# treangenlab/Seqwin

Hardware: AMD Instinct MI355X
Metric: Gbp/s minimizer-indexed (higher is better)
Workload: dtype u64

## Files before the change

### seqwin_amd/csrc/radix.hip

```cpp
#include <algorithm>
#include <cstdlib>
#include <cstring>
#include <vector>
#include <map>
#include <mutex>

#include "device.hpp"

namespace sw {
namespace {

constexpr int RS_ITEMS = 16;
#ifdef SW_RS_STAMPS
__device__ unsigned long long *g_rs_stamps = nullptr;
#define RS_STAMP(i)                                                                                        \
    do {                                                                                                   \
        if (g_rs_stamps && (tile & 63u) == 0 && threadIdx.x == 0) g_rs_stamps[(size_t)(tile >> 6) * 16 + (i)] = clock64(); \
    } while (0)
#else
#define RS_STAMP(i) do { } while (0)
#endif
#ifndef RS_LOOK
#define RS_LOOK 4
#endif
// ... 1098 lines not shown

bool radix_unsort_perm(uint64_t *&keys, uint64_t *&alt, uint64_t n, unsigned low_bits, unsigned nbit, hipStream_t stream, uint32_t *d_fail)
{
    constexpr int THREADS = 512, BITS = 8;
    constexpr uint32_t RADIX = 1u << BITS, TILE = THREADS * RS_ITEMS;
    if (n == 0 || nbit <= low_bits + 8 || nbit > low_bits + 16 || SW_AB_GETENV("SEQWIN_AMD_RADIX_STABLE_UNSORT")) return false;
    if ((1ull << (low_bits + 8)) % TILE) return false;
    const char *kind = SW_AB_GETENV("SEQWIN_AMD_RADIX_KERNEL");
    if (kind && !strcmp(kind, "classic")) return false;
    const unsigned hi_bits = nbit - low_bits - 8;
    const uint32_t n_groups = (uint32_t)((n + (1ull << (low_bits + 8)) - 1) >> (low_bits + 8));
    const uint64_t n_tiles = (n + TILE - 1) / TILE;
    int dev = 0, per_cu = 0;
    SW_HIP(hipGetDevice(&dev));
    hipDeviceProp_t prop;
    SW_HIP(hipGetDeviceProperties(&prop, dev));
    SW_HIP(hipOccupancyMaxActiveBlocksPerMultiprocessor(&per_cu, k_rs_pass_p<THREADS, BITS, 0>, THREADS, 0));
    const unsigned grid = (unsigned)std::min<uint64_t>(n_tiles, (uint64_t)std::max(1, per_cu) * std::max(1, prop.multiProcessorCount));
    DevArray<unsigned long long> cur_a((size_t)RADIX * RS_CURSOR_STRIDE), cur_b((size_t)n_groups * RADIX);
    DevArray<uint32_t> tickets(2);
    SW_HIP(hipMemsetAsync(tickets.p, 0, 8, stream));
    hipLaunchKernelGGL(k_rs_perm_cursors, dim3(1), dim3(RADIX), 0, stream, cur_a.p, 1u, RADIX, RS_CURSOR_STRIDE, 64u, low_bits + 8);
    hipLaunchKernelGGL(k_rs_perm_cursors, dim3((n_groups * RADIX + 255) / 256), dim3(256), 0, stream, cur_b.p, n_groups, RADIX, 1u,
                       low_bits + 8, low_bits);
    auto pass = ballot_forced() ? k_rs_pass_p<THREADS, BITS, 0> : k_rs_pass_p<THREADS, BITS, 1>;
    hipLaunchKernelGGL(pass, dim3(grid), dim3(THREADS), 0, stream, (const uint64_t *)keys, alt, n, (uint32_t)n_tiles,
                       32u + low_bits + 8, hi_bits, (const unsigned long long *)nullptr, (unsigned long long *)nullptr, tickets.p, d_fail,
                       0u, cur_a.p, RS_CURSOR_STRIDE, 64u, 0u);
    std::swap(keys, alt);
    hipLaunchKernelGGL(pass, dim3(grid), dim3(THREADS), 0, stream, (const uint64_t *)keys, alt, n, (uint32_t)n_tiles, 32u + low_bits,
                       8u, (const unsigned long long *)nullptr, (unsigned long long *)nullptr, tickets.p + 1, d_fail, 0u, cur_b.p, 1u,
                       low_bits + 8, 0u);
    std::swap(keys, alt);
    SW_HIP(hipGetLastError());
    return true;
}

bool radix_pairs_available() { return rank_mode() == 1; }
int radix_rank_mode() { return rank_mode(); }

uint64_t radix_trim_state()
{
    uint64_t freed = 0;
    if (g_state_uses) return 0;
    std::lock_guard<std::mutex> lock(state_registry_mu());
    for (auto &kv : state_registry()) {
        StateBuf &b = *kv.second;
        std::unique_lock<std::mutex> use(b.mu, std::try_to_lock);
        if (!use.owns_lock() || !b.p) continue;
        int cur = -1;
        (void)hipGetDevice(&cur);
        if (cur != kv.first.first) (void)hipSetDevice(kv.first.first);
        (void)hipFree(b.p);
        if (cur != kv.first.first && cur >= 0) (void)hipSetDevice(cur);
        freed += b.words * 8;
        b.p = nullptr;
        b.words = 0;
        b.epoch = 0;
    }
    return freed;
}

void radix_demote_rank()
{
    int dev = 0;
    SW_HIP(hipGetDevice(&dev));
    std::lock_guard<std::mutex> lock(rank_mu());
    rank_modes()[dev] = 0;
}

void radix_sort_pairs32(uint32_t *&keys, uint32_t *&keys_alt, OccPay *&vals, OccPay *&vals_alt, uint64_t n, unsigned end_bit,
                        hipStream_t stream, uint32_t *d_fail, const StageSource *src, const std::function<void()> &after_first,
                        uint32_t *low_out)
{
    constexpr uint32_t RADIX = 1u << RP_BITS, TILE = RP_THREADS * RP_ITEMS;
    if (n == 0 || end_bit == 0) return;
    if (end_bit > 32 || end_bit % RP_BITS) raise(SW_ERR_RUNTIME, "radix_sort_pairs32: key bits must be a multiple of 8 up to 32");
    if (n >= 0xFFFFFFFFull) raise(SW_ERR_RUNTIME, "radix_sort_pairs32: more than 2^32-2 elements");
    const unsigned n_passes = end_bit / RP_BITS;
    const uint64_t n_tiles = (n + TILE - 1) / TILE;
    int grid_p = 0;
    {
        static std::mutex &mu = *new std::mutex;
        static std::map<int, int> &grids = *new std::map<int, int>;
        int dev = 0;
        SW_HIP(hipGetDevice(&dev));
        std::lock_guard<std::mutex> lock(mu);
        int &g = grids[dev];
        if (!g) {
            int per_cu = 0;
            hipDeviceProp_t prop;
            SW_HIP(hipGetDeviceProperties(&prop, dev));
            SW_HIP(hipOccupancyMaxActiveBlocksPerMultiprocessor(&per_cu, k_rs_pair_pass<0>, RP_THREADS, 0));
            g = std::max(1, per_cu) * std::max(1, prop.multiProcessorCount);
        }
        grid_p = g;
    }
    DevArray<unsigned long long> hist((size_t)n_passes * RADIX);
    DevArray<uint32_t> tickets(n_passes);
    SW_HIP(hipMemsetAsync(tickets.p, 0, tickets.bytes(), stream));
    SW_HIP(hipMemsetAsync(hist.p, 0, hist.bytes(), stream));
    StageSource stage{};
    DevArray<uint32_t> chunk_tile;
    DevArray<unsigned long long> chunk_dir;
    if (src && src->rows) {
        stage = *src;
        hipLaunchKernelGGL(k_rs_hist32_rows, dim3((unsigned)((n + 16383) / 16384)), dim3(256), 0, stream,
                           reinterpret_cast<const uint4 *>(src->rows), n, n_passes, hist.p);
    } else if (src) {
        constexpr uint64_t CHUNK = 64 * RP_ITEMS;
        static_assert(TILE == (RP_THREADS / 64) * CHUNK, "a tile is one chunk per wave");
        const uint64_t n_chunks = (n + CHUNK - 1) / CHUNK;
        stage = *src;
        chunk_tile.alloc(n_chunks);
        chunk_dir.alloc(n_chunks * STAGE_ROW);
        stage.chunk_dir = chunk_dir.p;
        hipLaunchKernelGGL(k_rs_chunk_tiles, dim3((stage.n_tiles + 255u) / 256u), dim3(256), 0, stream, stage.tile_count, stage.dst_off,
                           stage.n_tiles, chunk_tile.p);
        hipLaunchKernelGGL(k_rs_stage_prepare, dim3((unsigned)std::min<uint64_t>(2048, (n_chunks + 3) / 4)), dim3(256), 0, stream, stage,
                           (const uint32_t *)chunk_tile.p, n, n_passes, chunk_dir.p, hist.p);
    } else {
        hipLaunchKernelGGL(k_rs_hist32, dim3((unsigned)((n + 65535) / 65536)), dim3(256), 0, stream, keys, n, n_passes, hist.p);
    }
    SW_HIP(hipGetLastError());
    StateUse su = state_buf(stream, (size_t)n_tiles * RADIX);
    StateBuf &sb = su.b;
    const StageSource none{};
    const uint32_t fault = fault_rank();
    for (unsigned p = 0; p < n_passes; ++p) {
        hipLaunchKernelGGL(k_rs_scan<RP_BITS>, dim3(1), dim3(RADIX), 0, stream, hist.p + (size_t)p * RADIX, (unsigned long long *)nullptr);
        const uint32_t epoch = next_epoch(sb, stream);
        const dim3 grid((unsigned)std::min<uint64_t>(n_tiles, (uint64_t)grid_p));
        if (p == 0 && src) {
            auto first = src->rows ? k_rs_pair_pass<2> : k_rs_pair_pass<1>;
            hipLaunchKernelGGL(first, grid, dim3(RP_THREADS), 0, stream, (const uint32_t *)nullptr, (const uint4 *)nullptr,
                               keys_alt, reinterpret_cast<uint4 *>(vals_alt), n, (uint32_t)n_tiles, 0u,
                               (const unsigned long long *)hist.p, sb.p, epoch, tickets.p, d_fail, stage,
                               n_passes == 1 ? low_out : (uint32_t *)nullptr, fault);
            SW_HIP(hipGetLastError());
            if (after_first) after_first();
        } else {
            hipLaunchKernelGGL(k_rs_pair_pass<0>, grid, dim3(RP_THREADS), 0, stream, (const uint32_t *)keys,
                               reinterpret_cast<const uint4 *>(vals), keys_alt, reinterpret_cast<uint4 *>(vals_alt), n, (uint32_t)n_tiles,
                               RP_BITS * p, (const unsigned long long *)(hist.p + (size_t)p * RADIX), sb.p, epoch, tickets.p + p, d_fail,
                               none, p + 1 == n_passes ? low_out : (uint32_t *)nullptr, fault);
            SW_HIP(hipGetLastError());
        }
        std::swap(keys, keys_alt);
        std::swap(vals, vals_alt);
    }
}

namespace {
constexpr uint32_t EB_RADIX = 512, EB_TABLE = EB_RADIX * EB_RADIX, EB_THREADS = 512;
constexpr uint64_t EB_EMPTY = ~0ull;
static_assert(EB_THREADS == EB_RADIX, "k_eb_finish: one bin per thread");
enum : uint32_t { EB_F_OVERFLOW = 1u, EB_F_RANGE = 2u, EB_F_ORDER = 4u };
struct EbInfo {
    unsigned long long n_sentinels;
    uint32_t n_tiles2, max_bucket, flags, n_runs;
};

__global__ __launch_bounds__(EB_RADIX) void k_eb_level1(const unsigned long long *__restrict__ h1, uint32_t tile_keys,
                                                        unsigned long long *__restrict__ cursor, unsigned long long *__restrict__ segtab,
                                                        EbInfo *__restrict__ info)
{
    __shared__ unsigned long long s[EB_RADIX];
    __shared__ uint32_t st[EB_RADIX];
    const uint32_t d = threadIdx.x;
    const unsigned long long c = h1[d];
    const uint32_t tiles = (uint32_t)((c + tile_keys - 1) / tile_keys);
    s[d] = c;
    st[d] = tiles;
    __syncthreads();
    for (uint32_t o = 1; o < EB_RADIX; o <<= 1) {
        const unsigned long long a = d >= o ? s[d - o] : 0;
        const uint32_t b = d >= o ? st[d - o] : 0;
        __syncthreads();
        s[d] += a;
        st[d] += b;
        __syncthreads();
    }
    const unsigned long long first = s[d] - c;
    cursor[(size_t)d * RS_CURSOR_STRIDE] = first;
    uint32_t w = st[d] - tiles;
    for (uint32_t t = 0; t < tiles; ++t)
        segtab[w + t] = seg_pack(first + (uint64_t)t * tile_keys, d, (uint32_t)min((unsigned long long)tile_keys, c - (uint64_t)t * tile_keys));
    if (d == EB_RADIX - 1) info->n_tiles2 = st[d];
}

__global__ __launch_bounds__(1024) void k_eb_count(const uint64_t *__restrict__ in, const unsigned long long *__restrict__ segtab,
                                                   const EbInfo *__restrict__ info, unsigned shift, uint32_t dmask, uint64_t sentinel,
                                                   uint32_t *__restrict__ table, EbInfo *__restrict__ out)
{
    __shared__ uint32_t hist[EB_RADIX];
    __shared__ uint32_t s_sent;
    const uint32_t n_tiles = info->n_tiles2;
    for (uint32_t w = blockIdx.x; w < n_tiles; w += gridDim.x) {
        const unsigned long long seg = segtab[w];
        const uint64_t first = seg_first(seg);
        const uint32_t cnt = seg_count(seg);
        if (threadIdx.x < EB_RADIX) hist[threadIdx.x] = 0;
        if (threadIdx.x == 0) s_sent = 0;
        __syncthreads();
        uint64_t key[RS_ITEMS];
#pragma unroll
        for (int i = 0; i < RS_ITEMS; ++i) {
            const uint32_t li = i * 1024 + threadIdx.x;
            key[i] = li < cnt ? in[first + li] : EB_EMPTY;
        }
        uint32_t sent = 0;
#pragma unroll
        for (int i = 0; i < RS_ITEMS; ++i) {
            if (key[i] == EB_EMPTY) continue;
            if (key[i] == sentinel) ++sent;
            atomicAdd(&hist[(uint32_t)(key[i] >> shift) & dmask], 1u);
        }
        if (sent) atomicAdd(&s_sent, sent);
        __syncthreads();
        if (threadIdx.x < EB_RADIX && hist[threadIdx.x]) atomicAdd(&table[seg_bucket(seg) * EB_RADIX + threadIdx.x], hist[threadIdx.x]);
        if (threadIdx.x == 0 && s_sent) atomicAdd(&out->n_sentinels, (unsigned long long)s_sent);
        __syncthreads();
    }
}

__global__ __launch_bounds__(1024) void k_eb_scan(const uint32_t *__restrict__ cnt, const unsigned long long *__restrict__ n_sent,
                                                  uint32_t sent_at, uint32_t *__restrict__ start, unsigned long long *__restrict__ cursor,
                                                  uint32_t *__restrict__ max_out, uint32_t *__restrict__ total_out)
{
    constexpr uint32_t PER4 = EB_TABLE / 1024 / 4;
    __shared__ uint32_t ws[16], wm[16];
    const uint32_t tid = threadIdx.x, lane = tid & 63u, wave = tid >> 6;
    const uint32_t sent = n_sent ? (uint32_t)*n_sent : 0u;
    const uint4 *cnt4 = reinterpret_cast<const uint4 *>(cnt) + (size_t)tid * PER4;
    uint32_t sum = 0, mx = 0;
#pragma unroll 16
    for (uint32_t j = 0; j < PER4; ++j) {
        const uint4 c = cnt4[j];
        mx = max(max(max(mx, c.x), max(c.y, c.z)), c.w);
        sum += c.x + c.y + c.z + c.w;
    }
    if (n_sent && sent_at / (4 * PER4) == tid) {
        mx = 0;
        for (uint32_t j = 0; j < 4 * PER4; ++j) {
            const uint32_t i = tid * 4 * PER4 + j, c = cnt[i];
            mx = max(mx, c - (i == sent_at ? min(c, sent) : 0u));
        }
    }
    uint32_t incl = sum;
    for (uint32_t o = 1; o < 64; o <<= 1) {
        const uint32_t up = __shfl_up(incl, o, 64);
        if (lane >= o) incl += up;
        mx = max(mx, __shfl_xor(mx, o, 64));
    }
    if (lane == 63) ws[wave] = incl;
    if (lane == 0) wm[wave] = mx;
    __syncthreads();
    uint32_t run = incl - sum;
    for (uint32_t w = 0; w < wave; ++w) run += ws[w];
    uint4 *start4 = reinterpret_cast<uint4 *>(start) + (size_t)tid * PER4;
    ulonglong2 *cur2 = reinterpret_cast<ulonglong2 *>(cursor) + (size_t)tid * PER4 * 2;
#pragma unroll 16
    for (uint32_t j = 0; j < PER4; ++j) {
        const uint4 c = cnt4[j];
        const uint4 st = make_uint4(run, run + c.x, run + c.x + c.y, run + c.x + c.y + c.z);
        start4[j] = st;
        if (cursor) {
            cur2[2 * j] = make_ulonglong2(st.x, st.y);
            cur2[2 * j + 1] = make_ulonglong2(st.z, st.w);
        }
        run = st.w + c.w;
    }
    if (tid == 1023) {
        start[EB_TABLE] = run;
        if (total_out) *total_out = run;
        uint32_t m = 0;
        for (uint32_t w = 0; w < 16; ++w) m = max(m, wm[w]);
        if (max_out) *max_out = m;
    }
}

__global__ __launch_bounds__(EB_THREADS) void k_eb_finish(const uint64_t *__restrict__ in, const uint32_t *__restrict__ start, uint32_t slots,
                                                          unsigned shift1, unsigned shift2, uint32_t mask2, unsigned bin_shift,
                                                          uint32_t bin_mask, uint64_t sentinel,
                                                          uint64_t *__restrict__ tk, uint32_t *__restrict__ tc,
                                                          uint32_t *__restrict__ n_distinct, uint32_t *__restrict__ flags)
{
    extern __shared__ __align__(16) unsigned char eb_lds[];
    unsigned long long *hk = reinterpret_cast<unsigned long long *>(eb_lds);
    uint32_t *hc = reinterpret_cast<uint32_t *>(hk + slots);
    uint16_t *idx = reinterpret_cast<uint16_t *>(hc + slots);
    __shared__ uint32_t bd[EB_RADIX + 1], bk[EB_RADIX], bcur[EB_RADIX], wsd[EB_THREADS / 64], wsk[EB_THREADS / 64];
    __shared__ uint32_t s_over;
    const uint32_t b = EB_TABLE - 1u - blockIdx.x, tid = threadIdx.x, lane = tid & 63u, wave = tid >> 6;
    const uint32_t first = start[b], cnt = start[b + 1] - first;
    if (cnt == 0) return;
    const uint32_t mask = slots - 1u;
    for (uint32_t s = tid; s < slots; s += EB_THREADS) {
        hk[s] = EB_EMPTY;
        hc[s] = 0;
    }
    bd[tid] = 0;
    bk[tid] = 0;
    if (tid == 0) s_over = 0;
    __syncthreads();
    uint32_t bad = 0;
    for (uint32_t j0 = 0; j0 < cnt; j0 += 4 * EB_THREADS) {
        if (*(volatile uint32_t *)&s_over) break;
        uint64_t key[4];
#pragma unroll
        for (int i = 0; i < 4; ++i) {
            const uint32_t j = j0 + i * EB_THREADS + tid;
            key[i] = j < cnt ? in[(uint64_t)first + j] : sentinel;
        }
#pragma unroll
        for (int i = 0; i < 4; ++i) {
            uint64_t k = key[i];
            bool live = k != sentinel;
            if (live && ((uint32_t)(k >> shift1) * EB_RADIX + ((uint32_t)(k >> shift2) & mask2)) != b) {
                bad = 1;
                live = false;
            }
            uint32_t copies = 1;
            const uint64_t any = __ballot(live);
            if (any) {
                const int src = __ffsll((long long)any) - 1;
                const uint64_t k0 = (uint64_t)__shfl((unsigned long long)k, src, 64);
                const uint64_t same = __ballot(live && k == k0);
                if (live && k == k0) {
                    copies = (uint32_t)__popcll(same);
                    live = (int)lane == src;
                }
            }
            if (!live) continue;
            uint32_t h = (uint32_t)((k * 0x9E3779B97F4A7C15ull) >> 40) & mask, probes = 0;
            for (; probes < slots; ++probes) {
                const unsigned long long old = atomicCAS(&hk[h], EB_EMPTY, (unsigned long long)k);
                if (old == EB_EMPTY || old == k) {
                    atomicAdd(&hc[h], copies);
                    break;
                }
                h = (h + 1u) & mask;
            }
            if (probes == slots) s_over = 1;
        }
    }
    if (bad) atomicOr(flags, EB_F_RANGE);
    __syncthreads();
    if (s_over) {
        if (tid == 0) atomicOr(flags, EB_F_OVERFLOW);
        return;
    }
    for (uint32_t s = tid; s < slots; s += EB_THREADS) {
        const uint64_t k = hk[s];
        if (k == EB_EMPTY) continue;
        const uint32_t bin = (uint32_t)(k >> bin_shift) & bin_mask;
        atomicAdd(&bd[bin], 1u);
        atomicAdd(&bk[bin], hc[s]);
    }
    __syncthreads();
    {
        const uint32_t d = bd[tid], c = bk[tid];
        uint32_t id = d, ic = c;
        for (uint32_t o = 1; o < 64; o <<= 1) {
            const uint32_t ud = __shfl_up(id, o, 64), uc = __shfl_up(ic, o, 64);
            if (lane >= o) {
                id += ud;
                ic += uc;
            }
        }
        if (lane == 63) {
            wsd[wave] = id;
            wsk[wave] = ic;
        }
        __syncthreads();
        uint32_t pd = id - d, pc = ic - c;
        for (uint32_t w = 0; w < wave; ++w) {
            pd += wsd[w];
            pc += wsk[w];
        }
        bd[tid] = pd;
        bcur[tid] = pd;
        bk[tid] = pc;
        if (tid == EB_THREADS - 1) bd[EB_RADIX] = pd + d;
    }
    __syncthreads();
    for (uint32_t s = tid; s < slots; s += EB_THREADS) {
        const uint64_t k = hk[s];
        if (k == EB_EMPTY) continue;
        idx[atomicAdd(&bcur[(uint32_t)(k >> bin_shift) & bin_mask], 1u)] = (uint16_t)s;
    }
    __syncthreads();
    const uint32_t n_dist = bd[EB_RADIX];
    if (tid == 0) n_distinct[b] = n_dist;
    for (uint32_t j = tid; j < n_dist; j += EB_THREADS) {
        const uint32_t s = idx[j];
        const uint64_t k = hk[s];
        const uint32_t bin = (uint32_t)(k >> bin_shift) & bin_mask, lo = bd[bin], hi = bd[bin + 1];
        uint32_t less = 0, copies_less = 0;
        for (uint32_t i = lo; i < hi; ++i) {
            const uint32_t s2 = idx[i];
            if (hk[s2] < k) {
                ++less;
                copies_less += hc[s2];
            }
        }
        tk[(uint64_t)first + lo + less] = k;
        tc[(uint64_t)first + lo + less] = first + bk[bin] + copies_less;
    }
}

__global__ __launch_bounds__(256) void k_eb_compact(const uint64_t *__restrict__ tk, const uint32_t *__restrict__ tc,
                                                    const uint32_t *__restrict__ start, const uint32_t *__restrict__ dstart,
                                                    const unsigned long long *__restrict__ n_sentinels, uint64_t *__restrict__ ukeys,
                                                    uint32_t *__restrict__ ucnt, uint32_t *__restrict__ flags)
{
    const uint32_t b = blockIdx.x, d0 = dstart[b], n = dstart[b + 1] - d0;
    if (b == EB_TABLE - 1u && threadIdx.x == 0) ucnt[dstart[EB_TABLE]] = start[EB_TABLE] - (uint32_t)*n_sentinels;
    if (n == 0) return;
    const uint64_t first = start[b];
    uint32_t bad = 0;
    for (uint32_t j = threadIdx.x; j < n; j += 256) {
        const uint64_t k = tk[first + j];
        const uint32_t c = tc[first + j];
        if (j + 1 < n && (tk[first + j + 1] <= k || tc[first + j + 1] <= c)) bad = 1;
        if (c < first || c >= start[b + 1]) bad = 1;
        ukeys[d0 + j] = k;
        ucnt[d0 + j] = c;
    }
    if (bad) atomicOr(flags, EB_F_ORDER);
}
}

int radix_edge_buckets(uint64_t *&keys, uint64_t *&alt, uint64_t m, unsigned key_bits, uint64_t sentinel,
                       const unsigned long long *d_hist_top, uint32_t cap, uint32_t slots, uint64_t *ukeys, uint32_t *ucnt,
                       uint32_t *n_runs, hipStream_t stream, uint32_t *d_fail, bool debug)
{
    constexpr int THREADS = 1024, BITS = 9;
    constexpr uint32_t TILE = THREADS * RS_ITEMS;
    unsigned digit_bits = 0, n_passes = 0;
    radix_layout(key_bits, &digit_bits, &n_passes);
    if (n_passes < 2 || m >= (1ull << 32) - 1 || slots < 64 || slots > 8192 || (slots & (slots - 1))) return 1;
    const unsigned shift1 = (n_passes - 1) * digit_bits, bits1 = key_bits - shift1;
    const unsigned bits2 = std::min<unsigned>(BITS, shift1), shift2 = shift1 - bits2;
    const unsigned bin_bits = std::min<unsigned>(BITS, shift2), bin_shift = shift2 - bin_bits;
    const uint64_t n_tiles = (m + TILE - 1) / TILE, max_tiles2 = n_tiles + EB_RADIX;
    int dev = 0, per_cu = 0;
    SW_HIP(hipGetDevice(&dev));
    hipDeviceProp_t prop;
    SW_HIP(hipGetDeviceProperties(&prop, dev));
    SW_HIP(hipOccupancyMaxActiveBlocksPerMultiprocessor(&per_cu, k_rs_pass_p<THREADS, BITS, 0>, THREADS, 0));
    const unsigned cus = (unsigned)std::max(1, prop.multiProcessorCount);
    const unsigned grid = (unsigned)std::min<uint64_t>(n_tiles, (uint64_t)std::max(1, per_cu) * cus);

    DevArray<unsigned long long> h1(EB_RADIX), cur1((size_t)EB_RADIX * RS_CURSOR_STRIDE), cur2(EB_TABLE), segtab(max_tiles2);
    DevArray<uint32_t> table(EB_TABLE), start(EB_TABLE + 1), tickets(2), flags(1);
    DevArray<EbInfo> info(1);
    SW_HIP(hipMemsetAsync(h1.p, 0, h1.bytes(), stream));
    SW_HIP(hipMemsetAsync(table.p, 0, table.bytes(), stream));
    SW_HIP(hipMemsetAsync(tickets.p, 0, 8, stream));
    SW_HIP(hipMemsetAsync(flags.p, 0, 4, stream));
    SW_HIP(hipMemsetAsync(info.p, 0, sizeof(EbInfo), stream));
    if (d_hist_top)
        SW_HIP(hipMemcpyAsync(h1.p, d_hist_top, (size_t)8 << digit_bits, hipMemcpyDeviceToDevice, stream));
    else
        hipLaunchKernelGGL(k_rs_hist<BITS>, dim3((unsigned)((m + 32767) / 32768)), dim3(256), 0, stream, (const uint64_t *)keys, m, shift1,
                           key_bits, 1u, h1.p);
    hipLaunchKernelGGL(k_eb_level1, dim3(1), dim3(EB_RADIX), 0, stream, (const unsigned long long *)h1.p, TILE, cur1.p, segtab.p, info.p);
    auto pass1 = ballot_forced() ? k_rs_pass_p<THREADS, BITS, 0> : k_rs_pass_p<THREADS, BITS, 1>;
    hipLaunchKernelGGL(pass1, dim3(grid), dim3(THREADS), 0, stream, (const uint64_t *)keys, alt, m, (uint32_t)n_tiles, shift1, bits1,
                       (const unsigned long long *)nullptr, (unsigned long long *)nullptr, tickets.p, d_fail, 0u, cur1.p, RS_CURSOR_STRIDE,
                       64u, 0u);
    std::swap(keys, alt);
    hipLaunchKernelGGL(k_eb_count, dim3((unsigned)std::min<uint64_t>(max_tiles2, (uint64_t)8 * cus)), dim3(1024), 0, stream,
                       (const uint64_t *)keys, (const unsigned long long *)segtab.p, (const EbInfo *)info.p, shift2, (1u << bits2) - 1u,
                       sentinel, table.p, info.p);
    const uint32_t sent_at = (uint32_t)(sentinel >> shift1) * EB_RADIX + ((uint32_t)(sentinel >> shift2) & ((1u << bits2) - 1u));
    hipLaunchKernelGGL(k_eb_scan, dim3(1), dim3(1024), 0, stream, (const uint32_t *)table.p, (const unsigned long long *)&info.p->n_sentinels,
                       sent_at, start.p, cur2.p, &info.p->max_bucket, (uint32_t *)nullptr);
    SW_HIP(hipGetLastError());
    EbInfo hi;
    SW_HIP(hipMemcpyAsync(&hi, info.p, sizeof hi, hipMemcpyDeviceToHost, stream));
    SW_HIP(hipStreamSynchronize(stream));
    if (debug)
        fprintf(stderr, "[edge buckets] %llu keys, %llu sentinels, digits %u+%u+%u of %u bits, largest sub-bucket %u (capacity %u, %u slots)%s\n",
                (unsigned long long)m, hi.n_sentinels, bits1, bits2, bin_bits, key_bits, hi.max_bucket, cap, slots,
                hi.max_bucket > cap ? ": radix passes instead" : "");
    if (hi.max_bucket > cap) return 1;
    auto pass2 = ballot_forced() ? k_rs_pass_p<THREADS, BITS, 0, true> : k_rs_pass_p<THREADS, BITS, 1, true>;
    hipLaunchKernelGGL(pass2, dim3(std::max(1u, std::min(hi.n_tiles2, (uint32_t)(std::max(1, per_cu) * cus)))), dim3(THREADS), 0, stream,
                       (const uint64_t *)keys, alt, m, hi.n_tiles2, shift2, bits2, (const unsigned long long *)segtab.p,
                       (unsigned long long *)nullptr, tickets.p + 1, d_fail, 0u, cur2.p, 1u, 64u, 0u);
    std::swap(keys, alt);
    DevArray<uint32_t> tc(m), n_distinct(EB_TABLE), dstart(EB_TABLE + 1);
    SW_HIP(hipMemsetAsync(n_distinct.p, 0, n_distinct.bytes(), stream));
    uint64_t *tk = alt;
    const size_t lds = (size_t)slots * 14;
    static std::mutex &mu = *new std::mutex;
    {
        std::lock_guard<std::mutex> lock(mu);
        SW_HIP(hipFuncSetAttribute(reinterpret_cast<const void *>(k_eb_finish), hipFuncAttributeMaxDynamicSharedMemorySize, (int)lds));
    }
    hipLaunchKernelGGL(k_eb_finish, dim3(EB_TABLE), dim3(EB_THREADS), lds, stream, (const uint64_t *)keys, (const uint32_t *)start.p, slots,
                       shift1, shift2, (1u << bits2) - 1u, bin_shift, (1u << bin_bits) - 1u, sentinel, tk, tc.p, n_distinct.p, flags.p);
    hipLaunchKernelGGL(k_eb_scan, dim3(1), dim3(1024), 0, stream, (const uint32_t *)n_distinct.p, (const unsigned long long *)nullptr, 0u,
                       dstart.p, (unsigned long long *)nullptr, (uint32_t *)nullptr, &info.p->n_runs);
    hipLaunchKernelGGL(k_eb_compact, dim3(EB_TABLE), dim3(256), 0, stream, (const uint64_t *)tk, (const uint32_t *)tc.p,
                       (const uint32_t *)start.p, (const uint32_t *)dstart.p, (const unsigned long long *)&info.p->n_sentinels, ukeys, ucnt,
                       flags.p);
    SW_HIP(hipGetLastError());
    uint32_t hf = 0;
    SW_HIP(hipMemcpyAsync(&hi, info.p, sizeof hi, hipMemcpyDeviceToHost, stream));
    SW_HIP(hipMemcpyAsync(&hf, flags.p, 4, hipMemcpyDeviceToHost, stream));
    SW_HIP(hipStreamSynchronize(stream));
    if (hf & (EB_F_RANGE | EB_F_ORDER))
        raise(SW_ERR_RUNTIME, "internal error: the edge buckets are out of order (%s)", hf & EB_F_RANGE ? "a key outside its bucket" : "run starts descend");
    if (hf & EB_F_OVERFLOW) {
        if (debug) fprintf(stderr, "[edge buckets] a sub-bucket holds more than %u distinct keys: radix passes instead\n", slots);
        return 1;
    }
    *n_runs = hi.n_runs;
    return 0;
}

static int pick_shape(unsigned bits)
{
    const char *e = SW_TEST_GETENV("SEQWIN_AMD_RADIX_BITS");
    const bool nine = e ? atoi(e) == 9 : (bits + 8) / 9 < (bits + 7) / 8;
    const char *shape = SW_AB_GETENV("SEQWIN_AMD_RADIX_SHAPE");
    if (shape && !strcmp(shape, "1024x8")) return 2;
    if (shape && !strcmp(shape, "512x9")) return 3;
    if (shape && !strcmp(shape, "256x8")) return 4;
    return nine ? 1 : 0;
}

void radix_layout(unsigned bits, unsigned *digit_bits, unsigned *n_passes)
{
    const int sh = pick_shape(bits);
    *digit_bits = (sh == 1 || sh == 3) ? 9u : 8u;
    *n_passes = (bits + *digit_bits - 1) / *digit_bits;
}

void radix_sort_keys64(uint64_t *&keys, uint64_t *&alt, uint64_t n, unsigned begin_bit, unsigned end_bit, hipStream_t stream,
                       uint32_t *d_fail, bool perm_hi32, unsigned long long *d_hist_given, unsigned layout_bits)
{
    if (n == 0 || end_bit <= begin_bit) return;
    if (end_bit - begin_bit > 64) raise(SW_ERR_RUNTIME, "radix_sort_keys64: more than 64 key bits");
    switch (pick_shape(layout_bits ? layout_bits : end_bit - begin_bit)) {
#ifdef SW_AB
    case 2: sort_passes<1024, 8>(keys, alt, n, begin_bit, end_bit, stream, d_fail, perm_hi32, d_hist_given); break;
    case 3: sort_passes<512, 9>(keys, alt, n, begin_bit, end_bit, stream, d_fail, perm_hi32, d_hist_given); break;
    case 4: sort_passes<256, 8>(keys, alt, n, begin_bit, end_bit, stream, d_fail, perm_hi32, d_hist_given); break;
#endif
    case 1: sort_passes<1024, 9>(keys, alt, n, begin_bit, end_bit, stream, d_fail, perm_hi32, d_hist_given); break;
    default: sort_passes<512, 8>(keys, alt, n, begin_bit, end_bit, stream, d_fail, perm_hi32, d_hist_given); break;
    }
}

}
```

Baseline: 474.5.

## Size edge-bucket finish hash tables by bucket class with persistent ticketed workgroups

```diff
diff --git a/seqwin_amd/csrc/radix.hip b/seqwin_amd/csrc/radix.hip
--- a/seqwin_amd/csrc/radix.hip
+++ b/seqwin_amd/csrc/radix.hip
@@ -1274,14 +1274,18 @@
 }
 
 namespace {
-constexpr uint32_t EB_RADIX = 512, EB_TABLE = EB_RADIX * EB_RADIX, EB_THREADS = 512;
+constexpr uint32_t EB_RADIX = 512, EB_TABLE = EB_RADIX * EB_RADIX;
 constexpr uint64_t EB_EMPTY = ~0ull;
-static_assert(EB_THREADS == EB_RADIX, "k_eb_finish: one bin per thread");
 enum : uint32_t { EB_F_OVERFLOW = 1u, EB_F_RANGE = 2u, EB_F_ORDER = 4u };
 struct EbInfo {
     unsigned long long n_sentinels;
     uint32_t n_tiles2, max_bucket, flags, n_runs;
 };
+constexpr uint32_t EB_MAX_CLASSES = 3;
+struct EbClasses {
+    uint32_t n, slots[EB_MAX_CLASSES], bound[EB_MAX_CLASSES], max_keys[EB_MAX_CLASSES];
+};
+enum : uint32_t { EB_CTL_COUNT = 0, EB_CTL_TICKET = 4, EB_CTL_PROMOTED = 8, EB_CTL_WORDS = 12 };
 
 __global__ __launch_bounds__(EB_RADIX) void k_eb_level1(const unsigned long long *__restrict__ h1, uint32_t tile_keys,
                                                         unsigned long long *__restrict__ cursor, unsigned long long *__restrict__ segtab,
@@ -1402,133 +1406,255 @@
     }
 }
 
-__global__ __launch_bounds__(EB_THREADS) void k_eb_finish(const uint64_t *__restrict__ in, const uint32_t *__restrict__ start, uint32_t slots,
-                                                          unsigned shift1, unsigned shift2, uint32_t mask2, unsigned bin_shift,
-                                                          uint32_t bin_mask, uint64_t sentinel,
-                                                          uint64_t *__restrict__ tk, uint32_t *__restrict__ tc,
-                                                          uint32_t *__restrict__ n_distinct, uint32_t *__restrict__ flags)
-{
+#ifdef SW_EB_STAMPS
+constexpr uint32_t EB_STAMP_N = 4096, EB_STAMP_W = 12;
+__device__ unsigned long long g_eb_stamps[EB_MAX_CLASSES][EB_STAMP_N][EB_STAMP_W];
+#define EB_STAMP_SET(t) const uint32_t stamp_at = ((t) & 15u) == 0 && ((t) >> 4) < EB_STAMP_N && threadIdx.x == 0 ? ((t) >> 4) : ~0u
+#define EB_STAMP(i) do { if (stamp_at != ~0u) g_eb_stamps[cls][stamp_at][i] = clock64(); } while (0)
+#define EB_STAMP_END(cnt, nd) do { if (stamp_at != ~0u) { g_eb_stamps[cls][stamp_at][9] = clock64(); g_eb_stamps[cls][stamp_at][10] = (cnt); g_eb_stamps[cls][stamp_at][11] = (nd); } } while (0)
+#else
+#define EB_STAMP_SET(t) do { } while (0)
+#define EB_STAMP(i) do { } while (0)
+#define EB_STAMP_END(cnt, nd) do { } while (0)
+#endif
+__global__ __launch_bounds__(1024) void k_eb_classify(const uint32_t *__restrict__ start, EbClasses cl, uint32_t force,
+                                                      uint4 *__restrict__ lists, uint32_t *__restrict__ ctl)
+{
+    const uint32_t b = (blockIdx.x ? blockIdx.x - 1u : gridDim.x - 1u) * 1024u + threadIdx.x, lane = threadIdx.x & 63u;
+    const uint32_t first = start[b], cnt = start[b + 1] - first;
+    uint32_t mine = EB_MAX_CLASSES;
+    if (cnt) {
+        mine = 0;
+        while (mine + 1 < cl.n && cnt > cl.max_keys[mine]) ++mine;
+        if (force < cl.n) mine = force;
+    }
+    for (uint32_t c = 0; c < cl.n; ++c) {
+        const uint64_t in = __ballot(mine == c);
+        if (!in) continue;
+        const int leader = __ffsll((long long)in) - 1;
+        uint32_t base = 0;
+        if ((int)lane == leader) base = atomicAdd(&ctl[EB_CTL_COUNT + c], (uint32_t)__popcll(in));
+        base = __shfl(base, leader, 64);
+        if (mine == c) lists[(size_t)c * EB_TABLE + base + (uint32_t)__popcll(in & ((1ull << lane) - 1ull))] = make_uint4(first, cnt, b, 0u);
+    }
+}
+
+template <int THREADS, bool ONE>
+__global__ __launch_bounds__(THREADS) void k_eb_finish(const uint64_t *__restrict__ in, uint4 *lists, uint32_t *__restrict__ ctl,
+                                                       uint32_t cls, EbClasses cl, unsigned shift1, unsigned shift2, uint32_t mask2,
+                                                       unsigned bin_shift, uint32_t bin_mask, unsigned cbits, uint64_t sentinel,
+                                                       uint64_t *__restrict__ tk, uint32_t *__restrict__ tc,
+                                                       uint32_t *__restrict__ n_distinct, uint32_t *__restrict__ flags)
+{
+    constexpr uint32_t BPT = EB_RADIX / THREADS, TILE = 4 * THREADS;
+    static_assert(BPT * THREADS == EB_RADIX, "k_eb_finish: whole bins per thread");
     extern __shared__ __align__(16) unsigned char eb_lds[];
+    const uint32_t slots = cl.slots[cls], bound = cl.bound[cls], mask = slots - 1u;
     unsigned long long *hk = reinterpret_cast<unsigned long long *>(eb_lds);
     uint32_t *hc = reinterpret_cast<uint32_t *>(hk + slots);
-    uint16_t *idx = reinterpret_cast<uint16_t *>(hc + slots);
-    __shared__ uint32_t bd[EB_RADIX + 1], bk[EB_RADIX], bcur[EB_RADIX], wsd[EB_THREADS / 64], wsk[EB_THREADS / 64];
-    __shared__ uint32_t s_over;
-    const uint32_t b = EB_TABLE - 1u - blockIdx.x, tid = threadIdx.x, lane = tid & 63u, wave = tid >> 6;
-    const uint32_t first = start[b], cnt = start[b + 1] - first;
-    if (cnt == 0) return;
-    const uint32_t mask = slots - 1u;
-    for (uint32_t s = tid; s < slots; s += EB_THREADS) {
-        hk[s] = EB_EMPTY;
-        hc[s] = 0;
-    }
-    bd[tid] = 0;
-    bk[tid] = 0;
-    if (tid == 0) s_over = 0;
-    __syncthreads();
-    uint32_t bad = 0;
-    for (uint32_t j0 = 0; j0 < cnt; j0 += 4 * EB_THREADS) {
-        if (*(volatile uint32_t *)&s_over) break;
-        uint64_t key[4];
+    uint16_t *idx = ONE ? reinterpret_cast<uint16_t *>(hk + slots) : reinterpret_cast<uint16_t *>(hc + slots);
+    __shared__ uint32_t bd[EB_RADIX + 1], bk[EB_RADIX], bcur[EB_RADIX], wsd[THREADS / 64], wsk[THREADS / 64];
+    __shared__ uint32_t s_over, s_ticket;
+    const uint32_t tid = threadIdx.x, lane = tid & 63u, wave = tid >> 6;
+    const uint64_t cmask = (1ull << cbits) - 1ull, low = (1ull << shift2) - 1ull;
+    auto slot_key = [&](uint32_t s) -> uint64_t { return ONE ? hk[s] >> cbits : hk[s]; };
+    auto slot_copies = [&](uint32_t s) -> uint32_t { return ONE ? (uint32_t)(hk[s] & cmask) : hc[s]; };
+    const uint4 *list = lists + (size_t)cls * EB_TABLE;
+    const uint32_t n_list = ctl[EB_CTL_COUNT + cls];
+    if (tid == 0) s_ticket = atomicAdd(&ctl[EB_CTL_TICKET + cls], 1u);
+    __syncthreads();
+    uint32_t t = s_ticket;
+    uint4 work = make_uint4(0u, 0u, 0u, 0u);
+    uint64_t key[4] = {sentinel, sentinel, sentinel, sentinel};
+    if (t < n_list) {
+        work = list[t];
 #pragma unroll
         for (int i = 0; i < 4; ++i) {
-            const uint32_t j = j0 + i * EB_THREADS + tid;
-            key[i] = j < cnt ? in[(uint64_t)first + j] : sentinel;
-        }
-#pragma unroll
-        for (int i = 0; i < 4; ++i) {
-            uint64_t k = key[i];
-            bool live = k != sentinel;
-            if (live && ((uint32_t)(k >> shift1) * EB_RADIX + ((uint32_t)(k >> shift2) & mask2)) != b) {
-                bad = 1;
-                live = false;
-            }
-            uint32_t copies = 1;
-            const uint64_t any = __ballot(live);
-            if (any) {
-                const int src = __ffsll((long long)any) - 1;
-                const uint64_t k0 = (uint64_t)__shfl((unsigned long long)k, src, 64);
-                const uint64_t same = __ballot(live && k == k0);
-                if (live && k == k0) {
-                    copies = (uint32_t)__popcll(same);
-                    live = (int)lane == src;
+            const uint32_t j = i * THREADS + tid;
+            key[i] = j < work.y ? in[(uint64_t)work.x + j] : sentinel;
+        }
+    }
+    __syncthreads();
+    while (t < n_list) {
+        const uint32_t first = work.x, cnt = work.y, b = work.z;
+        EB_STAMP_SET(t);
+        EB_STAMP(0);
+        const uint64_t high = ((uint64_t)(b / EB_RADIX) << shift1) | ((uint64_t)(b % EB_RADIX) << shift2);
+        for (uint32_t s = tid; s < slots; s += THREADS) {
+            hk[s] = EB_EMPTY;
+            if (!ONE) hc[s] = 0;
+        }
+#pragma unroll
+        for (uint32_t i = 0; i < BPT; ++i) {
+            bd[i * THREADS + tid] = 0;
+            bk[i * THREADS + tid] = 0;
+        }
+        if (tid == 0) {
+            s_over = 0;
+            s_ticket = atomicAdd(&ctl[EB_CTL_TICKET + cls], 1u);
+        }
+        __syncthreads();
+        EB_STAMP(1);
+        uint32_t bad = 0;
+        for (uint32_t j0 = 0;;) {
+#pragma unroll
+            for (int i = 0; i < 4; ++i) {
+                uint64_t k = key[i];
+                bool live = k != sentinel;
+                if (live && ((uint32_t)(k >> shift1) * EB_RADIX + ((uint32_t)(k >> shift2) & mask2)) != b) {
+                    bad = 1;
+                    live = false;
                 }
-            }
-            if (!live) continue;
-            uint32_t h = (uint32_t)((k * 0x9E3779B97F4A7C15ull) >> 40) & mask, probes = 0;
-            for (; probes < slots; ++probes) {
-                const unsigned long long old = atomicCAS(&hk[h], EB_EMPTY, (unsigned long long)k);
-                if (old == EB_EMPTY || old == k) {
-                    atomicAdd(&hc[h], copies);
-                    break;
+                uint32_t copies = 1;
+                const uint64_t any = __ballot(live);
+                if (any) {
+                    const int src = __ffsll((long long)any) - 1;
+                    const uint64_t k0 = (uint64_t)__shfl((unsigned long long)k, src, 64);
+                    const uint64_t same = __ballot(live && k == k0);
+                    if (live && k == k0) {
+                        copies = (uint32_t)__popcll(same);
+                        live = (int)lane == src;
+                    }
                 }
-                h = (h + 1u) & mask;
-            }
-            if (probes == slots) s_over = 1;
-        }
-    }
-    if (bad) atomicOr(flags, EB_F_RANGE);
-    __syncthreads();
-    if (s_over) {
-        if (tid == 0) atomicOr(flags, EB_F_OVERFLOW);
-        return;
-    }
-    for (uint32_t s = tid; s < slots; s += EB_THREADS) {
-        const uint64_t k = hk[s];
-        if (k == EB_EMPTY) continue;
-        const uint32_t bin = (uint32_t)(k >> bin_shift) & bin_mask;
-        atomicAdd(&bd[bin], 1u);
-        atomicAdd(&bk[bin], hc[s]);
-    }
-    __syncthreads();
-    {
-        const uint32_t d = bd[tid], c = bk[tid];
-        uint32_t id = d, ic = c;
-        for (uint32_t o = 1; o < 64; o <<= 1) {
-            const uint32_t ud = __shfl_up(id, o, 64), uc = __shfl_up(ic, o, 64);
-            if (lane >= o) {
-                id += ud;
-                ic += uc;
-            }
-        }
-        if (lane == 63) {
-            wsd[wave] = id;
-            wsk[wave] = ic;
-        }
+                if (!live) continue;
+                uint32_t h = (uint32_t)((k * 0x9E3779B97F4A7C15ull) >> 40) & mask, probes = 0;
+                if (ONE) {
+                    const uint64_t rem = k & low;
+                    const unsigned long long fresh = (unsigned long long)((rem << cbits) | copies);
+                    for (; probes < slots; ++probes) {
+                        const unsigned long long old = atomicCAS(&hk[h], EB_EMPTY, fresh);
+                        if (old == EB_EMPTY) break;
+                        if ((old >> cbits) == rem) {
+                            atomicAdd(&hk[h], (unsigned long long)copies);
+                            break;
+                        }
+                        h = (h + 1u) & mask;
+                    }
+                } else {
+                    for (; probes < slots; ++probes) {
+                        const unsigned long long old = atomicCAS(&hk[h], EB_EMPTY, (unsigned long long)k);
+                        if (old == EB_EMPTY || old == k) {
+                            atomicAdd(&hc[h], copies);
+                            break;
+                        }
+                        h = (h + 1u) & mask;
+                    }
+                }
+                if (probes == slots) s_over = 1;
+            }
+            j0 += TILE;
+            if (j0 >= cnt || *(volatile uint32_t *)&s_over) break;
+#pragma unroll
+            for (int i = 0; i < 4; ++i) {
+                const uint32_t j = j0 + i * THREADS + tid;
+                key[i] = j < cnt ? in[(uint64_t)first + j] : sentinel;
+            }
+        }
+        if (bad) atomicOr(flags, EB_F_RANGE);
+        EB_STAMP(2);
         __syncthreads();
-        uint32_t pd = id - d, pc = ic - c;
-        for (uint32_t w = 0; w < wave; ++w) {
-            pd += wsd[w];
-            pc += wsk[w];
-        }
-        bd[tid] = pd;
-        bcur[tid] = pd;
-        bk[tid] = pc;
-        if (tid == EB_THREADS - 1) bd[EB_RADIX] = pd + d;
-    }
-    __syncthreads();
-    for (uint32_t s = tid; s < slots; s += EB_THREADS) {
-        const uint64_t k = hk[s];
-        if (k == EB_EMPTY) continue;
-        idx[atomicAdd(&bcur[(uint32_t)(k >> bin_shift) & bin_mask], 1u)] = (uint16_t)s;
-    }
-    __syncthreads();
-    const uint32_t n_dist = bd[EB_RADIX];
-    if (tid == 0) n_distinct[b] = n_dist;
-    for (uint32_t j = tid; j < n_dist; j += EB_THREADS) {
-        const uint32_t s = idx[j];
-        const uint64_t k = hk[s];
-        const uint32_t bin = (uint32_t)(k >> bin_shift) & bin_mask, lo = bd[bin], hi = bd[bin + 1];
-        uint32_t less = 0, copies_less = 0;
-        for (uint32_t i = lo; i < hi; ++i) {
-            const uint32_t s2 = idx[i];
-            if (hk[s2] < k) {
-                ++less;
-                copies_less += hc[s2];
-            }
-        }
-        tk[(uint64_t)first + lo + less] = k;
-        tc[(uint64_t)first + lo + less] = first + bk[bin] + copies_less;
+        EB_STAMP(3);
+        t = s_ticket;
+        if (t < n_list) work = list[t];
+        bool redo = s_over != 0;
+        uint32_t n_dist = 0;
+        if (!redo) {
+            for (uint32_t s = tid; s < slots; s += THREADS) {
+                if (hk[s] == EB_EMPTY) continue;
+                const uint32_t bin = (uint32_t)(slot_key(s) >> bin_shift) & bin_mask;
+                atomicAdd(&bd[bin], 1u);
+                atomicAdd(&bk[bin], slot_copies(s));
+            }
+            __syncthreads();
+            EB_STAMP(4);
+            {
+                uint32_t d[BPT], c[BPT], sd = 0, sc = 0;
+#pragma unroll
+                for (uint32_t i = 0; i < BPT; ++i) {
+                    d[i] = bd[tid * BPT + i];
+                    c[i] = bk[tid * BPT + i];
+                    sd += d[i];
+                    sc += c[i];
+                }
+                uint32_t id = sd, ic = sc;
+                for (uint32_t o = 1; o < 64; o <<= 1) {
+                    const uint32_t ud = __shfl_up(id, o, 64), uc = __shfl_up(ic, o, 64);
+                    if (lane >= o) {
+                        id += ud;
+                        ic += uc;
+                    }
+                }
+                if (lane == 63) {
+                    wsd[wave] = id;
+                    wsk[wave] = ic;
+                }
+                __syncthreads();
+                uint32_t pd = id - sd, pc = ic - sc;
+                for (uint32_t w = 0; w < wave; ++w) {
+                    pd += wsd[w];
+                    pc += wsk[w];
+                }
+#pragma unroll
+                for (uint32_t i = 0; i < BPT; ++i) {
+                    bd[tid * BPT + i] = pd;
+                    bcur[tid * BPT + i] = pd;
+                    bk[tid * BPT + i] = pc;
+                    pd += d[i];
+                    pc += c[i];
+                }
+                if (tid == THREADS - 1) bd[EB_RADIX] = pd;
+            }
+            __syncthreads();
+            EB_STAMP(5);
+            n_dist = bd[EB_RADIX];
+            redo = n_dist > bound;
+        }
+        if (!redo) {
+            for (uint32_t s = tid; s < slots; s += THREADS) {
+                if (hk[s] == EB_EMPTY) continue;
+                idx[atomicAdd(&bcur[(uint32_t)(slot_key(s) >> bin_shift) & bin_mask], 1u)] = (uint16_t)s;
+            }
+            __syncthreads();
+        }
+        EB_STAMP(6);
+        if (t < n_list) {
+#pragma unroll
+            for (int i = 0; i < 4; ++i) {
+                const uint32_t j = i * THREADS + tid;
+                key[i] = j < work.y ? in[(uint64_t)work.x + j] : sentinel;
+            }
+        }
+        EB_STAMP(7);
+        if (redo) {
+            if (tid == 0) {
+                if (cls + 1 < cl.n) {
+                    lists[(size_t)(cls + 1) * EB_TABLE + atomicAdd(&ctl[EB_CTL_COUNT + cls + 1], 1u)] = make_uint4(first, cnt, b, 0u);
+                    atomicAdd(&ctl[EB_CTL_PROMOTED + cls], 1u);
+                } else {
+                    atomicOr(flags, EB_F_OVERFLOW);
+                }
+            }
+        } else {
+            if (tid == 0) n_distinct[b] = n_dist;
+            for (uint32_t j = tid; j < n_dist; j += THREADS) {
+                const uint32_t s = idx[j];
+                const uint64_t k = slot_key(s);
+                const uint32_t bin = (uint32_t)(k >> bin_shift) & bin_mask, lo = bd[bin], hi = bd[bin + 1];
+                uint32_t less = 0, copies_less = 0;
+                for (uint32_t i = lo; i < hi; ++i) {
+                    const uint32_t s2 = idx[i];
+                    if (slot_key(s2) < k) {
+                        ++less;
+                        copies_less += slot_copies(s2);
+                    }
+                }
+                tk[(uint64_t)first + lo + less] = ONE ? (high | k) : k;
+                tc[(uint64_t)first + lo + less] = first + bk[bin] + copies_less;
+            }
+        }
+        EB_STAMP(8);
+        __syncthreads();
+        EB_STAMP_END(cnt, n_dist);
     }
 }
 
@@ -1553,6 +1679,61 @@
     if (bad) atomicOr(flags, EB_F_ORDER);
 }
 }
+
+#ifdef SW_EB_STAMPS
+#define EB_STAMPS_BEGIN() do { void *sp = nullptr; SW_HIP(hipGetSymbolAddress(&sp, HIP_SYMBOL(g_eb_stamps))); SW_HIP(hipMemsetAsync(sp, 0, sizeof g_eb_stamps, stream)); } while (0)
+#define EB_STAMPS_REPORT() eb_stamps_report(cl, start.p, n_distinct.p)
+static void eb_stamps_report(const EbClasses &cl, const uint32_t *d_start, const uint32_t *d_ndist)
+{
+    static const char *phase[9] = {"clear", "keys", "barrier", "bins", "scan", "place", "prefetch", "rank+store", "barrier"};
+    std::vector<unsigned long long> st((size_t)EB_MAX_CLASSES * EB_STAMP_N * EB_STAMP_W);
+    SW_HIP(hipMemcpyFromSymbol(st.data(), HIP_SYMBOL(g_eb_stamps), st.size() * 8));
+    for (uint32_t c = 0; c < cl.n; ++c) {
+        double sum[9] = {}, keys = 0, nd = 0;
+        uint32_t n = 0;
+        for (uint32_t i = 0; i < EB_STAMP_N; ++i) {
+            const unsigned long long *r = &st[((size_t)c * EB_STAMP_N + i) * EB_STAMP_W];
+            if (!r[9] || !r[11]) continue;
+            for (int p = 0; p < 9; ++p) sum[p] += (double)(r[p + 1] - r[p]);
+            keys += (double)r[10];
+            nd += (double)r[11];
+            ++n;
+        }
+        fprintf(stderr, "[eb stamps] class %u (%u slots): %u samples, mean keys %.0f distinct %.0f, ticks", c, cl.slots[c], n, n ? keys / n : 0, n ? nd / n : 0);
+        double total = 0;
+        for (int p = 0; p < 9; ++p) {
+            fprintf(stderr, " %s %.0f", phase[p], n ? sum[p] / n : 0);
+            total += n ? sum[p] / n : 0;
+        }
+        fprintf(stderr, " total %.0f\n", total);
+    }
+    std::vector<uint32_t> hs(EB_TABLE + 1), hd(EB_TABLE);
+    SW_HIP(hipMemcpy(hs.data(), d_start, hs.size() * 4, hipMemcpyDeviceToHost));
+    SW_HIP(hipMemcpy(hd.data(), d_ndist, hd.size() * 4, hipMemcpyDeviceToHost));
+    uint32_t hk[24] = {}, hdd[24] = {};
+    double bk[16] = {}, bdd[16] = {};
+    uint32_t bn[16] = {};
+    for (uint32_t b = 0; b < EB_TABLE; ++b) {
+        const uint32_t k = hs[b + 1] - hs[b];
+        if (!k) continue;
+        ++hk[std::min(23u, k / 1024)];
+        ++hdd[std::min(23u, hd[b] / 256)];
+        bk[b / 16384] += k;
+        bdd[b / 16384] += hd[b];
+        ++bn[b / 16384];
+    }
+    fprintf(stderr, "[eb hist] keys per non-empty sub-bucket, bins of 1024:");
+    for (uint32_t v : hk) fprintf(stderr, " %u", v);
+    fprintf(stderr, "\n[eb hist] distinct keys per non-empty sub-bucket, bins of 256:");
+    for (uint32_t v : hdd) fprintf(stderr, " %u", v);
+    fprintf(stderr, "\n[eb hist] per block of 16384 sub-buckets: non-empty, mean keys, mean distinct, keys/distinct:");
+    for (int i = 0; i < 16; ++i) fprintf(stderr, " [%u %.0f %.0f %.2f]", bn[i], bn[i] ? bk[i] / bn[i] : 0, bn[i] ? bdd[i] / bn[i] : 0, bdd[i] ? bk[i] / bdd[i] : 0);
+    fprintf(stderr, "\n");
+}
+#else
+#define EB_STAMPS_BEGIN() do { } while (0)
+#define EB_STAMPS_REPORT() do { } while (0)
+#endif
 
 int radix_edge_buckets(uint64_t *&keys, uint64_t *&alt, uint64_t m, unsigned key_bits, uint64_t sentinel,
                        const unsigned long long *d_hist_top, uint32_t cap, uint32_t slots, uint64_t *ukeys, uint32_t *ucnt,
@@ -1614,17 +1795,77 @@
                        (const uint64_t *)keys, alt, m, hi.n_tiles2, shift2, bits2, (const unsigned long long *)segtab.p,
                        (unsigned long long *)nullptr, tickets.p + 1, d_fail, 0u, cur2.p, 1u, 64u, 0u);
     std::swap(keys, alt);
-    DevArray<uint32_t> tc(m), n_distinct(EB_TABLE), dstart(EB_TABLE + 1);
+    const uint32_t mask2v = (1u << bits2) - 1u, bin_maskv = (1u << bin_bits) - 1u;
+    DevArray<uint32_t> tc(m), n_distinct(EB_TABLE), dstart(EB_TABLE + 1), ctl(EB_CTL_WORDS);
     SW_HIP(hipMemsetAsync(n_distinct.p, 0, n_distinct.bytes(), stream));
+    SW_HIP(hipMemsetAsync(ctl.p, 0, ctl.bytes(), stream));
     uint64_t *tk = alt;
-    const size_t lds = (size_t)slots * 14;
-    static std::mutex &mu = *new std::mutex;
+    const unsigned cbits = 32u - (unsigned)__builtin_clz(cap + 1u);
+    bool one_word = shift2 + cbits <= 64;
+    uint32_t small_slots[EB_MAX_CLASSES - 1] = {1024, 2048}, keys_per_distinct = 4, force = EB_MAX_CLASSES;
+    if (const char *e = SW_TEST_GETENV("SEQWIN_AMD_EDGE_FINISH_SIZES")) {
+        small_slots[0] = (uint32_t)strtoul(e, nullptr, 10);
+        small_slots[1] = strchr(e, ',') ? (uint32_t)strtoul(strchr(e, ',') + 1, nullptr, 10) : 0u;
+    }
+    uint32_t small_bound[EB_MAX_CLASSES - 1] = {0, 0};
+    if (const char *e = SW_TEST_GETENV("SEQWIN_AMD_EDGE_FINISH_BOUNDS")) {
+        small_bound[0] = (uint32_t)strtoul(e, nullptr, 10);
+        small_bound[1] = strchr(e, ',') ? (uint32_t)strtoul(strchr(e, ',') + 1, nullptr, 10) : 0u;
+    }
+    if (const char *e = SW_TEST_GETENV("SEQWIN_AMD_EDGE_FINISH_RATIO")) keys_per_distinct = std::max(1u, (uint32_t)strtoul(e, nullptr, 10));
+    if (const char *e = SW_TEST_GETENV("SEQWIN_AMD_EDGE_FINISH_CLASS")) force = (uint32_t)strtoul(e, nullptr, 10);
+    if (const char *e = SW_TEST_GETENV("SEQWIN_AMD_EDGE_FINISH_WIDE")) one_word = one_word && atoi(e) == 0;
+    EbClasses cl{};
+    for (uint32_t i = 0; i + 1 < EB_MAX_CLASSES; ++i) {
+        const uint32_t s = small_slots[i];
+        if (s >= 64 && !(s & (s - 1)) && s < slots && (cl.n == 0 || s > cl.slots[cl.n - 1])) {
+            cl.slots[cl.n] = s;
+            cl.bound[cl.n] = small_bound[i] ? std::min(small_bound[i], s) : s / 8 * 5;
+            cl.max_keys[cl.n] = cl.bound[cl.n] * keys_per_distinct;
+            ++cl.n;
+        }
+    }
+    cl.slots[cl.n] = slots;
+    cl.bound[cl.n] = slots;
+    if (const char *e = SW_TEST_GETENV("SEQWIN_AMD_EDGE_FINISH_LAST_BOUND")) cl.bound[cl.n] = std::min(slots, (uint32_t)strtoul(e, nullptr, 10));
+    cl.max_keys[cl.n] = ~0u;
+    ++cl.n;
+    force = force < EB_MAX_CLASSES ? std::min(force, cl.n - 1u) : cl.n;
+    DevArray<uint4> lists((size_t)cl.n * EB_TABLE);
+    hipLaunchKernelGGL(k_eb_classify, dim3(EB_TABLE / 1024), dim3(1024), 0, stream, (const uint32_t *)start.p, cl, force, lists.p, ctl.p);
+    auto pick = [&](bool last) -> const void * {
+        if (last) return one_word ? reinterpret_cast<const void *>(k_eb_finish<512, true>) : reinterpret_cast<const void *>(k_eb_finish<512, false>);
+        return one_word ? reinterpret_cast<const void *>(k_eb_finish<256, true>) : reinterpret_cast<const void *>(k_eb_finish<256, false>);
+    };
+    const size_t slot_bytes = one_word ? 10 : 14;
+    int occ[EB_MAX_CLASSES] = {};
     {
+        static std::mutex &mu = *new std::mutex;
+        static std::map<const void *, size_t> limit;
+        static std::map<std::pair<const void *, size_t>, int> occupancy;
         std::lock_guard<std::mutex> lock(mu);
-        SW_HIP(hipFuncSetAttribute(reinterpret_cast<const void *>(k_eb_finish), hipFuncAttributeMaxDynamicSharedMemorySize, (int)lds));
-    }
-    hipLaunchKernelGGL(k_eb_finish, dim3(EB_TABLE), dim3(EB_THREADS), lds, stream, (const uint64_t *)keys, (const uint32_t *)start.p, slots,
-                       shift1, shift2, (1u << bits2) - 1u, bin_shift, (1u << bin_bits) - 1u, sentinel, tk, tc.p, n_distinct.p, flags.p);
+        for (uint32_t c = 0; c < cl.n; ++c) {
+            const void *fn = pick(c + 1 == cl.n);
+            const size_t lds = cl.slots[c] * slot_bytes;
+            size_t &lim = limit[fn];
+            if (lds > lim) {
+                SW_HIP(hipFuncSetAttribute(fn, hipFuncAttributeMaxDynamicSharedMemorySize, (int)lds));
+                lim = lds;
+            }
+            int &o = occupancy[{fn, lds}];
+            if (!o) SW_HIP(hipOccupancyMaxActiveBlocksPerMultiprocessor(&o, fn, c + 1 == cl.n ? 512 : 256, lds));
+            occ[c] = o;
+        }
+    }
+    EB_STAMPS_BEGIN();
+    for (uint32_t c = 0; c < cl.n; ++c) {
+        const bool last = c + 1 == cl.n;
+        const unsigned wgs = (unsigned)std::max(1, occ[c]) * cus;
+        void *args[] = {(void *)&keys, (void *)&lists.p, (void *)&ctl.p, (void *)&c, (void *)&cl, (void *)&shift1, (void *)&shift2, (void *)&mask2v,
+                        (void *)&bin_shift, (void *)&bin_maskv, (void *)&cbits, (void *)&sentinel, (void *)&tk, (void *)&tc.p, (void *)&n_distinct.p,
+                        (void *)&flags.p};
+        SW_HIP(hipLaunchKernel(pick(last), dim3(wgs), dim3(last ? 512 : 256), args, cl.slots[c] * slot_bytes, stream));
+    }
     hipLaunchKernelGGL(k_eb_scan, dim3(1), dim3(1024), 0, stream, (const uint32_t *)n_distinct.p, (const unsigned long long *)nullptr, 0u,
                        dstart.p, (unsigned long long *)nullptr, (uint32_t *)nullptr, &info.p->n_runs);
     hipLaunchKernelGGL(k_eb_compact, dim3(EB_TABLE), dim3(256), 0, stream, (const uint64_t *)tk, (const uint32_t *)tc.p,
@@ -1634,7 +1875,16 @@
     uint32_t hf = 0;
     SW_HIP(hipMemcpyAsync(&hi, info.p, sizeof hi, hipMemcpyDeviceToHost, stream));
     SW_HIP(hipMemcpyAsync(&hf, flags.p, 4, hipMemcpyDeviceToHost, stream));
+    uint32_t hc[EB_CTL_WORDS] = {};
+    if (debug) SW_HIP(hipMemcpyAsync(hc, ctl.p, sizeof hc, hipMemcpyDeviceToHost, stream));
     SW_HIP(hipStreamSynchronize(stream));
+    if (debug) {
+        fprintf(stderr, "[edge finish] %s slots, classes", one_word ? "one-word" : "two-array");
+        for (uint32_t c = 0; c < cl.n; ++c)
+            fprintf(stderr, " %u:%u+%u", cl.slots[c], hc[EB_CTL_COUNT + c] - (c ? hc[EB_CTL_PROMOTED + c - 1] : 0u), c + 1 < cl.n ? hc[EB_CTL_PROMOTED + c] : 0u);
+        fprintf(stderr, "\n");
+    }
+    EB_STAMPS_REPORT();
     if (hf & (EB_F_RANGE | EB_F_ORDER))
         raise(SW_ERR_RUNTIME, "internal error: the edge buckets are out of order (%s)", hf & EB_F_RANGE ? "a key outside its bucket" : "run starts descend");
     if (hf & EB_F_OVERFLOW) {
```

Measured after the change: 488.1 (median of 6 runs). 2.9% higher.
